# rileyhales/river-route

Hardware: AMD Instinct MI355X
Metric: reach-steps/sec (higher is better)
Workload: dtype f64

## Files before the change

### river_route_amd/csrc/rr_kernels_rec.hpp

```cpp
#pragma once

namespace {

constexpr int kRecCols = 32, kRecBatch = 8, kRecThreads = 256;
constexpr int kRecInThreads = kRecThreads, kRecOutThreads = kRecThreads;
constexpr int kRecInCols = kRecCols, kRecOutCols = kRecCols;
constexpr int kRecRows = 16 * kRecBatch;
constexpr int kRecLaunchBatches = 4, kRecMaxLaunchBatches = 8;

struct RecPermArgs {
    double *rec;
    Div32 rec_chunks;
    int64_t n, np, T, total, batch;
    Div32 nsub;
    const int2 *colmeta;
    const double *scale;
    RowView rows;
    const float *rows_in32;
    float *rows32;
    Div32 factor;
    const int32_t *cols;
    int32_t swizzle;
    int32_t clamp;
    uint32_t in32_sel, out32_sel;
// ... 23 lines not shown

constexpr int kRecTileRows = 16 * kRecBatch + 15;
constexpr int kRecTileLd = kRecCols + 1;

__device__ __forceinline__ uint32_t ring_chunk(const Div32 &chunks, uint32_t first, uint32_t ahead)
{
    const uint32_t c = first + ahead;
    return c >= chunks.d ? c - chunks.d : c;
}

template <bool SUB, int THREADS = kRecThreads, int BATCH = kRecBatch, bool LDSMETA = false, int COLS = kRecCols>
__device__ __forceinline__ void write_records(const RecPermArgs &a, const double *tile, int64_t col0, int64_t batch, int64_t tick_first, int64_t row_first,
                                              const int2 *smeta = nullptr, const double *sscale = nullptr)
{
    constexpr int R = 16 * BATCH + 15;
    const int tid = threadIdx.x;
    static_assert(COLS * BATCH * 8 % THREADS == 0, "records of a tile must divide among the threads");
    constexpr int IT = COLS * BATCH * 8 / THREADS;
    int2 meta[LDSMETA ? 1 : IT];
    double f[LDSMETA ? 1 : IT];
    if constexpr (!LDSMETA) {
#pragma unroll
        for (int it = 0; it < IT; ++it) {
            const int64_t i = col0 + (it * THREADS + tid) / (8 * BATCH);
            meta[it] = i < a.n ? a.colmeta[i] : make_int2(-1, 0);
        }
#pragma unroll
        for (int it = 0; it < IT; ++it) {
            const int64_t i = col0 + (it * THREADS + tid) / (8 * BATCH);
            f[it] = (a.scale && i < a.n) ? a.scale[i] : 1.0;
        }
    }
    const uint32_t chunk_first = a.rec_chunks.mod((uint32_t)kRecBatch * (uint32_t)batch);
#pragma unroll(LDSMETA ? (SUB ? 2 : 4) : IT)
    for (int it = 0; it < IT; ++it) {
        const int piece = it * THREADS + tid;
        const int c = piece / (8 * BATCH), k = (piece >> 3) % BATCH, part = piece & 7;
        const int2 m = LDSMETA ? smeta[c] : meta[LDSMETA ? 0 : it];
        const double scale = LDSMETA ? sscale[c] : f[LDSMETA ? 0 : it];
        const int32_t p = m.x;
        if (p < 0) continue;
        const int32_t lag = m.y & kLagMask;
        const int o = lag & 15;
        const uint32_t chunk = ring_chunk(a.rec_chunks, chunk_first, (uint32_t)(lag >> 4) + k);
        const int r = 15 - o + 16 * k + 2 * part;
        double v0, v1;
        if (SUB) {
            const int64_t t0 = tick_first + r, t1 = t0 + 1;
            uint32_t s;
            const int r0 = t0 < 0 ? 0 : (int)((int64_t)a.nsub.div((uint32_t)t0, s) - row_first);
            const int r1 = t1 < 0 ? 0 : (int)((int64_t)a.nsub.div((uint32_t)t1, s) - row_first);
            v0 = tile[min(r0, R - 1) * (COLS + 1) + c] * scale; v1 = tile[min(r1, R - 1) * (COLS + 1) + c] * scale;
        } else {
            v0 = tile[r * (COLS + 1) + c] * scale; v1 = tile[(r + 1) * (COLS + 1) + c] * scale;
        }
        double2 *dst = reinterpret_cast<double2 *>(a.rec + rec_elem(chunk, a.np, p)) + part;
        typedef double d2 __attribute__((ext_vector_type(2)));
        *reinterpret_cast<d2 *>(dst) = d2{v0, v1};
    }
}

template <bool SUB, bool IN32 = false, bool ENS = false, bool HW = false>
__global__ __launch_bounds__(kRecInThreads, 4) void k_rec_in(const RecArgsOf<ENS> args)
{
    static_assert(!HW || (!SUB && !ENS), "headwaters are routed by the in-pass only with one sub-step per row, single member");
    const RecPermArgs &a = member_args(args);
    constexpr int R = kRecTileRows, G = kRecInThreads / kRecInCols;
    __shared__ double tile[R * (kRecInCols + 1)];
    __shared__ int2 smeta[kRecInCols];
    __shared__ double sscale[kRecInCols];
    __shared__ double shw[5][HW ? kRecInCols : 1];
    const int tid = threadIdx.x;
    auto first_row = [&](int64_t tick_first) -> int64_t {
        uint32_t sub_unused;
        return SUB ? (int64_t)a.nsub.div((uint32_t)(tick_first < 0 ? 0 : tick_first), sub_unused) : tick_first;
    };
    int64_t tick_first = kRecRows * a.batch - 15;
    int64_t row_first = first_row(tick_first);
    constexpr int RPT = (R + G - 1) / G;
    const int c = tid % kRecInCols, r0 = tid / kRecInCols;
    const int need = SUB ? (int)((uint32_t)(R - 1) / a.nsub.d) + 2 : R;
    const uint32_t n_tiles = (uint32_t)((a.n + kRecInCols - 1) / kRecInCols);
    if (blockIdx.x >= n_tiles) return;
    const int64_t col0 = (int64_t)(a.swizzle ? xcd_swizzle(blockIdx.x, n_tiles) : blockIdx.x) * kRecInCols;
    const int64_t i = min(col0 + c, a.n - 1);
    const bool live = col0 + c < a.n;
    auto load = [&](int64_t t) -> double {
        const int64_t off = a.rows.offset(t < 0 ? 0 : (t >= a.T ? a.T - 1 : t)) + i;
        return IN32 ? (double)f32_from_file(a.rows_in32[off], a.in32_sel) : a.rows.base[off];
    };
    {
        double v[RPT];
        int2 cm = make_int2(-1, 0);
        double cs = 1.0;
        double hc1 = 0.0, hc2 = 0.0, hc3 = 0.0, hq = 0.0;
        if (tid < kRecInCols) {
            cm = live ? a.colmeta[i] : make_int2(-1, 0);
            cs = a.scale ? a.scale[i] : 1.0;
            if constexpr (HW) {
                hc1 = a.hw_coef[3 * i]; hc2 = a.hw_coef[3 * i + 1]; hc3 = a.hw_coef[3 * i + 2];
                hq = a.hw_carry[i];
            }
        }
#pragma unroll
        for (int q = 0; q < RPT; ++q) v[q] = load(row_first + min(r0 + q * G, need - 1));
#pragma unroll
        for (int q = 0; q < RPT; ++q) {
            const int r = r0 + q * G;
            const int64_t row = row_first + r;
            if (r < R) tile[r * (kRecInCols + 1) + c] = (row >= 0 && row < a.T && live) ? v[q] : 0.0;
        }
        if (tid < kRecInCols) {
            smeta[c] = cm; sscale[c] = cs;
            if constexpr (HW) { shw[0][c] = hc1; shw[1][c] = hc2; shw[2][c] = hc3; shw[3][c] = hq; shw[4][c] = (cm.y & kColInpass) ? 1.0 : cs; }
        }
    }
    __syncthreads();
    auto route_headwaters = [&](int64_t first) {
        if (tid >= kRecInCols) return;
        const int2 m = smeta[tid];
        if (m.x < 0 || !(m.y & kColInpass)) return;
        const double c1 = shw[0][tid], c2 = shw[1][tid], c3 = shw[2][tid], sc = sscale[tid];
        double q = shw[3][tid];
        const int r_first = 15 - (m.y & 15);
        double *col = tile + r_first * (kRecInCols + 1) + tid;
        const int64_t t_first = first + r_first;
        constexpr int kBlk = 8;
#pragma unroll 1
        for (int b = 0; b < kRecRows; b += kBlk) {
            double x[kBlk];
#pragma unroll
            for (int k = 0; k < kBlk; ++k) x[k] = col[(b + k) * (kRecInCols + 1)] * sc;
            const int64_t t0 = t_first + b;
            if (t0 >= 0 && t0 + kBlk <= a.T) {
#pragma unroll
                for (int k = 0; k < kBlk; ++k) { q = __builtin_fma(c1, 0.0, __builtin_fma(c2, 0.0, __builtin_fma(c3, q, x[k]))); x[k] = q; }
            } else {
#pragma unroll
                for (int k = 0; k < kBlk; ++k) {
                    const bool in = t0 + k >= 0 && t0 + k < a.T;
                    const double qn = __builtin_fma(c1, 0.0, __builtin_fma(c2, 0.0, __builtin_fma(c3, q, x[k])));
                    q = in ? qn : q; x[k] = in ? qn : x[k];
                }
            }
#pragma unroll
            for (int k = 0; k < kBlk; ++k) col[(b + k) * (kRecInCols + 1)] = x[k];
        }
        shw[3][tid] = q;
    };
    const double *wscale = HW ? shw[4] : sscale;
    if constexpr (HW) { route_headwaters(tick_first); __syncthreads(); }
    const int nb = a.batches > 1 ? a.batches : 1;
    for (int b = 1; b < nb; ++b) {
        constexpr int NPT = kRecRows / G, KPT = 3;
        const int64_t tick_next = tick_first + kRecRows, row_next = first_row(tick_next);
        const int shift = (int)(row_next - row_first), keep = max(need - shift, 0);
        double v[NPT], kv[KPT];
#pragma unroll
        for (int q = 0; q < NPT; ++q) {
            const int r = keep + r0 + q * G;
            if (r < need) v[q] = load(row_next + r);
        }
        write_records<SUB, kRecInThreads, kRecBatch, true, kRecInCols>(a, tile, col0, a.batch + b - 1, tick_first, row_first, smeta, wscale);
#pragma unroll
        for (int q = 0; q < KPT; ++q) {
            const int r = r0 + q * G;
            if (r < keep) kv[q] = tile[(shift + r) * (kRecInCols + 1) + c];
        }
        __syncthreads();
#pragma unroll
        for (int q = 0; q < KPT; ++q) {
            const int r = r0 + q * G;
            if (r < keep) tile[r * (kRecInCols + 1) + c] = kv[q];
        }
#pragma unroll
        for (int q = 0; q < NPT; ++q) {
            const int r = keep + r0 + q * G;
            const int64_t row = row_next + r;
            if (r < need) tile[r * (kRecInCols + 1) + c] = (row >= 0 && row < a.T && live) ? v[q] : 0.0;
        }
        __syncthreads();
        tick_first = tick_next; row_first = row_next;
        if constexpr (HW) { route_headwaters(tick_first); __syncthreads(); }
    }
    if constexpr (HW) {
        if (tid < kRecInCols && live && (smeta[tid].y & kColInpass)) a.hw_carry[i] = shw[3][tid];
    }
    write_records<SUB, kRecInThreads, kRecBatch, true, kRecInCols>(a, tile, col0, a.batch + nb - 1, tick_first, row_first, smeta, wscale);
}

struct UhArgs {
    const double *kernel, *state;
    int32_t n_ks;
};
constexpr int kUhCols = 16, kUhTileLd = kUhCols + 1;
constexpr int kUhMaxBatches = 2;
constexpr int uh_threads(int batches) { return 32 * kRecBatch * batches; }
constexpr int uh_tile_rows(int batches) { return 16 * kRecBatch * batches + 15; }
constexpr int uh_groups(int batches) { return uh_threads(batches) / kUhCols; }
constexpr int uh_rows_per_thread(int batches) { return (uh_tile_rows(batches) + uh_groups(batches) - 1) / uh_groups(batches); }
constexpr int uh_win_rows(int batches) { return uh_groups(batches) * uh_rows_per_thread(batches); }
constexpr size_t rec_in_uh_lds_bytes(int nk, int batches) { return (size_t)((uh_win_rows(batches) + nk - 1) + nk) * kUhTileLd * sizeof(double); }

template <bool SUB, int NK, int BATCHES, bool IN32 = false>
__global__ __launch_bounds__(uh_threads(BATCHES)) void k_rec_in_uh(const RecPermArgs a, const UhArgs u)
{
    constexpr int R = uh_tile_rows(BATCHES), G = uh_groups(BATCHES), RP = uh_rows_per_thread(BATCHES);
    constexpr int ROWS = uh_win_rows(BATCHES) + NK - 1, DATA = R + NK - 1;
    extern __shared__ __attribute__((aligned(16))) double uh_lds[];
    double *dt = uh_lds;
    double *tp = uh_lds + ROWS * kUhTileLd;
    const int tid = threadIdx.x, c = tid % kUhCols, g = tid / kUhCols;
    const int64_t col0 = (int64_t)(a.swizzle ? xcd_swizzle(blockIdx.x, gridDim.x) : blockIdx.x) * kUhCols;
    const int64_t tick_first = kRecRows * a.batch - 15;
    uint32_t sub_unused;
    const int64_t row_first = SUB ? (int64_t)a.nsub.div((uint32_t)(tick_first < 0 ? 0 : tick_first), sub_unused) : tick_first;
    const int need = SUB ? (int)((uint32_t)(R - 1) / a.nsub.d) + 2 : R;
    const int64_t i = min(col0 + c, a.n - 1);
    const bool live = col0 + c < a.n;
    const int32_t tb = (int32_t)row_first - (NK - 1) + g;
    {
// ... 206 lines not shown
```

### river_route_amd/csrc/rr_engine.hip

```cpp
#include "rr_common.hpp"
#include "rr_kernels_tick.hpp"
#include "rr_kernels_tile.hpp"
#include "rr_kernels_uh.hpp"
#include "rr_kernels_rec.hpp"
#include "rr_kernels_runoff.hpp"
#include "rr_kernels_direct.hpp"
#include "rr_kernels_metrics.hpp"
#include "rr_kernels_overlap.hpp"
#include "rr_kernels_adjoint.hpp"
#include "rr_kernels_adjoint_unit.hpp"
#include "rr_exec.hpp"


extern "C" {

int rr_version(void) { return RR_VERSION_NUM; }

const char *rr_last_error(void) { return g_err.c_str(); }

int rr_device_count(void)
{
    int c = 0;
    if (hipGetDeviceCount(&c) != hipSuccess) return 0;
    return c;
// ... 144 lines not shown
    info[0] = P->h.n; info[1] = P->h.n_edges; info[2] = P->h.depth; info[3] = P->h.widest_level;
    info[4] = P->h.n_headwaters; info[5] = P->h.n_outlets; info[6] = P->h.identity ? 1 : 0; info[7] = P->device;
    return RR_OK;
}

int rr_plan_layout(const rr_plan *P, int32_t *perm, int32_t *lag, int32_t *child_ptr)
{
    if (!P) return fail(RR_E_INVALID, "rr_plan_layout: null plan");
    const size_t n = (size_t)P->h.n;
    if (perm && n) std::memcpy(perm, P->h.perm.data(), n * sizeof(int32_t));
    if (lag && n) std::memcpy(lag, P->h.lag.data(), n * sizeof(int32_t));
    if (child_ptr) std::memcpy(child_ptr, P->h.child_ptr.data(), (n + 1) * sizeof(int32_t));
    return RR_OK;
}

int rr_plan_tile_info(const rr_plan *P, int64_t info[8])
{
    if (!P || !info) return fail(RR_E_INVALID, "rr_plan_tile_info: null argument");
    const rr::TilePlan &T = P->tp;
    info[0] = T.ok ? 1 : 0; info[1] = T.block; info[2] = T.np; info[3] = T.n_ghost; info[4] = T.n_tiles; info[5] = T.n_levels;
    info[6] = P->wave_threads; info[7] = kRecRows;
    return RR_OK;
}

int rr_plan_inpass_info(const rr_plan *P, int64_t info[5])
{
    if (!P || !info) return fail(RR_E_INVALID, "rr_plan_inpass_info: null argument");
    for (int k = 0; k < 5; ++k) info[k] = 0;
    info[0] = P->hw_inpass ? 1 : 0;
    if (!P->tp.ok) return RR_OK;
    std::vector<int32_t> lag(P->tp.lag);
    for (int32_t i : P->ghost_reach) lag[P->tp.inv[i]] |= kGhostBit;
    std::vector<uint8_t> elig;
    rr::mark_inpass_headwaters(P->tp, lag, kGhostBit, elig, info + 1);
    return RR_OK;
}

int rr_plan_tile_layout(const rr_plan *P, int32_t *tile_ptr, int32_t *tile_level, int32_t *perm, int32_t *lag, int32_t *cfirst,
                        uint32_t *ccnt, int32_t *xpos)
{
    if (!P) return fail(RR_E_INVALID, "rr_plan_tile_layout: null plan");
    const rr::TilePlan &T = P->tp;
    if (!T.ok) return fail(RR_E_UNSUPPORTED, "rr_plan_tile_layout: this network does not tile (a reach has more upstream reaches than a tile holds)");
    auto copy = [](auto *dst, const auto &src) { if (dst && !src.empty()) std::memcpy(dst, src.data(), src.size() * sizeof(src[0])); };
    copy(tile_ptr, T.tile_ptr); copy(tile_level, T.tile_level); copy(perm, T.perm); copy(lag, T.lag); copy(cfirst, T.cfirst);
    copy(ccnt, T.ccnt); copy(xpos, T.xpos);
    return RR_OK;
}

int rr_plan_direct_info(const rr_plan *P, int64_t info[8], char *why, int64_t why_cap)
{
    if (!P || !info) return fail(RR_E_INVALID, "rr_plan_direct_info: null argument");
    const rr::DirectPlan &D = P->dp;
    info[0] = D.ok ? 1 : 0; info[1] = D.n_tiles; info[2] = D.n_holes; info[3] = D.n_exports; info[4] = D.skel.np; info[5] = D.skel.n_tiles;
    info[6] = D.skel.n_levels; info[7] = P->direct_window;
    if (why && why_cap > 0) { std::strncpy(why, D.why.c_str(), (size_t)why_cap - 1); why[why_cap - 1] = 0; }
    return RR_OK;
}

int rr_plan_direct_layout(const rr_plan *P, int32_t *tile_c0, int32_t *tile_nc, int32_t *tile_lag_lo, int32_t *tile_span, int32_t *delay, int32_t *up3, int32_t *xinfo)
{
    if (!P) return fail(RR_E_INVALID, "rr_plan_direct_layout: null plan");
    const rr::DirectPlan &D = P->dp;
    if (!D.ok) return fail(RR_E_UNSUPPORTED, "rr_plan_direct_layout: the direct row path does not apply to this plan: " + D.why);
    auto copy = [](auto *dst, const auto &src) { if (dst && !src.empty()) std::memcpy(dst, src.data(), src.size() * sizeof(src[0])); };
    copy(tile_c0, D.tile_c0); copy(tile_nc, D.tile_nc); copy(tile_lag_lo, D.tile_lag_lo); copy(tile_span, D.tile_span);
    copy(delay, D.delay); copy(up3, D.up3); copy(xinfo, D.xinfo);
// ... 27 lines not shown
    int rc = need_device(P);
    if (rc) return rc;
    const rr::HostPlan &H = P->h;
    const int64_t n = H.n;
    if (n > 0 && (!c2 || !c3 || (H.n_edges > 0 && !lhs_off_data)))
        return fail(RR_E_INVALID, "rr_plan_set_coeffs: null coefficient array");
    std::vector<double> w(n), a2(n), a3(n), a4(n, 0.0);
    for (int64_t p = 0; p < n; ++p) {
        const int32_t i = H.perm[p];
        const int32_t e = H.edge_of[i];
        w[p] = e >= 0 ? -lhs_off_data[e] : 0.0;
        a2[p] = c2[i];
        a3[p] = c3[i];
        if (c4_dt) a4[p] = c4_dt[i];
    }
    std::vector<double> c1row(n, 0.0);
    bool uniform = true;
    for (int64_t p = 0; p < n; ++p) {
        const int32_t u0 = H.child_ptr[p], u1 = H.child_ptr[p + 1];
        if (u1 > u0) c1row[p] = w[u0];
        for (int32_t u = u0 + 1; u < u1; ++u) if (w[u] != w[u0]) uniform = false;
    }
    P->weights_uniform = uniform;
    rc = dev_upload(P->d_w, w);
    if (!rc) rc = dev_upload(P->d_c1row_h, c1row);
    if (!rc && P->tp.ok) {
        const rr::TilePlan &TP = P->tp;
        P->h_coef.assign(3 * TP.np, 0.0);
        for (int64_t p = 0; p < TP.np; ++p) {
            if (TP.lag[p] & kTileGhostBit) continue;
            const int32_t i = TP.perm[p];
            P->h_coef[3 * p] = c1row[H.inv[i]]; P->h_coef[3 * p + 1] = c2[i]; P->h_coef[3 * p + 2] = c3[i];
        }
        rc = upload_tile_coef(P);
    }
    {
        P->h_dcoef.assign(4 * (size_t)n, 0.0);
        for (int64_t i = 0; i < n; ++i) { P->h_dcoef[4 * i] = c1row[H.inv[i]]; P->h_dcoef[4 * i + 1] = c2[i]; P->h_dcoef[4 * i + 2] = c3[i]; P->h_dcoef[4 * i + 3] = c4_dt ? c4_dt[i] : 0.0; }
        if (!rc) rc = upload_direct_coef(P);
    }
    if (!rc) rc = dev_upload(P->d_c2, a2);
    if (!rc) rc = dev_upload(P->d_c3, a3);
    if (!rc) rc = dev_upload(P->d_c4, a4);
    if (!rc && c4_dt && n > 0) {
        hipError_t e = hipMemcpy(P->d_c4_params, c4_dt, (size_t)n * sizeof(double), hipMemcpyHostToDevice);
        if (e != hipSuccess) rc = fail(RR_E_HIP, hipGetErrorString(e));
    }
    if (rc) return rc;
    P->coeffs_set = true;
    P->has_c4 = c4_dt != nullptr;
    return RR_OK;
}

int rr_plan_set_unit_weights(rr_plan *P, const double *c1, const double *a_data)
{
    int rc = need_device(P);
    if (rc) return rc;
    if (P->ses.open) return fail(RR_E_STATE, "rr_plan_set_unit_weights: a routing call is open");
    if (!c1 && !a_data) { P->unit_general = false; return RR_OK; }
    const rr::HostPlan &H = P->h;
    const int64_t n = H.n;
    if (!c1 || (H.n_edges > 0 && !a_data)) return fail(RR_E_INVALID, "rr_plan_set_unit_weights: give both arrays, or neither to go back to unit weights");
    if (P->n_ghost > 0 || P->n_export > 0) return fail(RR_E_UNSUPPORTED, "rr_plan_set_unit_weights: general edge data on a partitioned network is not supported");
    std::vector<double> a2(n, 0.0), own(n, 0.0);
    for (int64_t p = 0; p < n; ++p) {
        const int32_t i = H.perm[p], e = H.edge_of[i];
        a2[p] = e >= 0 ? a_data[e] : 0.0;
// ... 1236 lines not shown
```

### river_route_amd/csrc/rr_exec.hpp

```cpp
#pragma once


enum class Mode { Rapid, Muskingum, Unit };

struct Rows {
    const double *dev_in = nullptr;
    const float *dev_in32 = nullptr;
    const double *host_in = nullptr;
    int64_t rows_in = 0;
    double *dev_out = nullptr;
    double *host_out = nullptr;
    int64_t rows_out = 0;
    float *dev_out32 = nullptr;
    int64_t out_factor = 1;
    const double *uh_kernel = nullptr, *uh_state = nullptr;
    int64_t uh_nks = 0;
    const RunoffArgs *runoff = nullptr;
    int64_t members = 0, in_pitch = 0, out_pitch = 0;
};

struct CallShape {
    Mode mode = Mode::Rapid;
    int64_t T = 0, nsub = 1;
    bool host = false;
// ... 88 lines not shown
    int32_t *d_bidx = nullptr;
    uint16_t *d_hwc = nullptr;
    double *d_w = nullptr, *d_c1row_h = nullptr, *d_c2 = nullptr, *d_c3 = nullptr, *d_c4 = nullptr;
    double *d_x = nullptr, *d_isum = nullptr, *d_qch = nullptr;
    double *d_a2 = nullptr, *d_c1own = nullptr, *d_z = nullptr;
    bool unit_general = false;
    double *d_ring = nullptr;
    int64_t ring_cap = 0;
    double *d_stage = nullptr;
    int64_t stage_cap = 0;
    double *d_mrows = nullptr;
    int64_t mrows_cap = 0;
    uint16_t *d_slot_a[2] = {nullptr, nullptr}, *d_slot_b[2] = {nullptr, nullptr};
    int32_t *d_m_index[2] = {nullptr, nullptr};
    int64_t perm_rows_per_block = 2;

    rr::TilePlan tp;
    bool wave_enabled = true, wave_forced = false, weights_uniform = false;
    bool ens_enabled = true;
    int wave_threads = 512;
    int64_t wave_K = 0;
    Schedule sch;
    int64_t kc_cap = int64_t{1} << 20;
    TileMeta *d_tmeta = nullptr;
    int4 *d_pmeta = nullptr;
    int32_t *d_tperm = nullptr, *d_tinv = nullptr;
    int32_t *d_inner_idx = nullptr;
    bool export_inside = false;
    double *d_coef = nullptr;
    double *d_coef_unit = nullptr;
    bool hw_inpass = true;
    std::vector<uint8_t> hw_elig;
    int64_t hw_counts[4] = {0, 0, 0, 0};
    int4 *d_pmeta_hw = nullptr;
    double *d_coef_hw = nullptr;
    double *d_hwcoef = nullptr;
    double *d_hwq = nullptr;
    std::vector<double> h_coef;
    int32_t n_wide_tiles = 0;
    double *d_sq = nullptr, *d_ss = nullptr, *d_si = nullptr, *d_sqch = nullptr;
    double *d_esq = nullptr, *d_ess = nullptr, *d_esi = nullptr;
    int64_t ens_cap = 0;
    double *d_full = nullptr, *d_chan = nullptr;
    int2 *d_colmeta = nullptr;
    int2 *d_ghostmeta = nullptr;
    double *d_c4_params = nullptr;
    size_t dev_total_bytes = 0;
    int cu_count = 256;

    int64_t n_ghost = 0, n_export = 0;
    int64_t ghost_min_lag = 0, export_max_lag = 0;
    std::vector<int32_t> ghost_reach, export_reach;

    Session ses;
    HostPipe pipe;
    rr::DirectPlan dp;
    bool direct_enabled = true;
    bool uh_rows_ok = true;
    int direct_window = 1;
    DirectTile *d_dtiles = nullptr;
    int4 *d_dlane = nullptr;
    int32_t *d_dsend_ptr = nullptr, *d_dsend_lane = nullptr;
    double *d_dcoef = nullptr, *d_dq = nullptr;
    TileMeta *d_ktmeta = nullptr;
    int4 *d_kpmeta = nullptr;
    int32_t *d_kperm = nullptr, *d_kholecol = nullptr;
// ... 48 lines not shown
int need_device(const rr_plan *plan)
{
    if (!plan) return fail(RR_E_INVALID, "null plan");
    if (plan->device < 0)
        return fail(RR_E_NO_DEVICE, "this plan is host-only (RR_DEVICE_NONE): the HIP engine has no CPU fallback");
    HIPCHK(hipSetDevice(plan->device));
    return RR_OK;
}

template <typename T>
int ensure_cap(T **buf, int64_t *cap, int64_t count)
{
    if (*cap >= count) return RR_OK;
    if (*buf) { (void)hipFree(*buf); *buf = nullptr; *cap = 0; }
    int rc = dev_alloc(buf, count);
    if (rc) return rc;
    *cap = count;
    return RR_OK;
}

int upload_tile_meta(rr_plan *P, const std::vector<int32_t> &lag, const std::vector<int32_t> &xpos, const std::vector<int32_t> &flags)
{
    const rr::TilePlan &TP = P->tp;
    std::vector<TileMeta> tm((size_t)TP.n_tiles);
    for (int32_t t = 0; t < TP.n_tiles; ++t)
        tm[t] = TileMeta{TP.tile_ptr[t], TP.tile_ptr[t + 1], TP.tile_level[t], TP.tile_lag_lo[t], TP.tile_lag_hi[t], flags[t], 0, 0};
    std::vector<int4> pm((size_t)TP.np);
    for (int64_t p = 0; p < TP.np; ++p) pm[p] = make_int4(lag[p], TP.cfirst[p], xpos[p], (int32_t)TP.ccnt[p]);
    int rc = RR_OK;
    if (!P->d_tmeta) rc = dev_alloc(&P->d_tmeta, TP.n_tiles);
    if (!rc && !P->d_pmeta) rc = dev_alloc(&P->d_pmeta, TP.np);
    if (!rc) rc = dev_upload(P->d_tmeta, tm);
    if (!rc) rc = dev_upload(P->d_pmeta, pm);
    rr::mark_inpass_headwaters(TP, lag, kGhostBit, P->hw_elig, P->hw_counts);
    if (!P->hw_inpass) { P->hw_elig.assign((size_t)TP.np, 0); P->hw_counts[0] = 0; }
    for (int64_t p = 0; p < TP.np; ++p) if (P->hw_elig[p]) pm[p].x |= kTileGhostBit;
    const rr::HostPlan &H = P->h;
    std::vector<int2> cm((size_t)H.n);
    for (int64_t i = 0; i < H.n; ++i)
        cm[i] = make_int2(TP.inv[i], (TP.lag[TP.inv[i]] & kLagMask) | (H.child_ptr[H.inv[i] + 1] == H.child_ptr[H.inv[i]] ? kColHeadwater : 0) |
                                         (P->hw_elig[TP.inv[i]] ? kColInpass : 0));
    if (!rc && !P->d_pmeta_hw) rc = dev_alloc(&P->d_pmeta_hw, TP.np);
    if (!rc) rc = dev_upload(P->d_pmeta_hw, pm);
    if (!rc && !P->d_colmeta) rc = dev_alloc(&P->d_colmeta, H.n);
    if (!rc) rc = dev_upload(P->d_colmeta, cm);
    return rc;
}

int upload_tile_coef(rr_plan *P)
{
    if (P->h_coef.empty()) return RR_OK;
    std::vector<double> coef(P->h_coef);
    for (int32_t i : P->ghost_reach) { const int64_t p = P->tp.inv[i]; coef[3 * p] = coef[3 * p + 1] = coef[3 * p + 2] = 0.0; }
    int rc = dev_upload(P->d_coef, coef);
    if (rc) return rc;
    {
        std::vector<double> hw(coef);
        for (int64_t p = 0; p < P->tp.np; ++p)
            if (P->hw_elig[p]) hw[3 * p] = hw[3 * p + 1] = hw[3 * p + 2] = 0.0;
        rc = dev_upload(P->d_coef_hw, hw);
        if (rc) return rc;
        std::vector<double> col(3 * (size_t)P->h.n);
        for (int64_t i = 0; i < P->h.n; ++i) for (int k = 0; k < 3; ++k) col[3 * i + k] = coef[3 * (int64_t)P->tp.inv[i] + k];
        rc = dev_upload(P->d_hwcoef, col);
        if (rc) return rc;
    }
    for (int64_t p = 0; p < P->tp.np; ++p)
// ... 1364 lines not shown
```

### river_route_amd/csrc/rr_plan.cpp

```cpp
#include "rr_plan.hpp"

#include <algorithm>
#include <cstdlib>
#include <limits>
#include <utility>
#include <vector>

#include "../../include/rr_hip.h"

namespace rr {

void build_tiled_permutation(const int32_t *pi, int64_t n, int32_t tile, TiledPermutation &T)
{
    T = TiledPermutation();
    T.n = n;
    T.tile = tile;
    if (n == 0) return;
    const int64_t nt = (n + tile - 1) / tile;
    std::vector<int32_t> q_of(n);
    for (int64_t q = 0; q < n; ++q) q_of[pi[q]] = (int32_t)q;
    std::vector<int64_t> run(nt * nt + 1, 0);
    for (int64_t i = 0; i < n; ++i) ++run[(int64_t)(q_of[i] / tile) * nt + i / tile + 1];
    for (size_t k = 1; k < run.size(); ++k) run[k] += run[k - 1];
    std::vector<int32_t> g_of(n);
    for (int64_t i = 0; i < n; ++i) g_of[i] = (int32_t)run[(int64_t)(q_of[i] / tile) * nt + i / tile]++;
    T.slot_a.resize(n); T.m_index.resize(n); T.slot_b.resize(n);
    std::vector<std::pair<int32_t, int32_t>> tmp;
    for (int64_t a = 0; a < nt; ++a) {
        const int64_t i0 = a * tile, i1 = std::min<int64_t>(n, i0 + tile);
        tmp.clear();
        for (int64_t i = i0; i < i1; ++i) tmp.emplace_back(g_of[i], (int32_t)i);
        std::sort(tmp.begin(), tmp.end());
        for (size_t m = 0; m < tmp.size(); ++m) {
            T.slot_a[tmp[m].second] = (uint16_t)m;
            T.m_index[i0 + (int64_t)m] = tmp[m].first;
        }
// ... 290 lines not shown
                    if (is_hw(c) != (pass == 0)) continue;
                    const bool ghost = tile_of_reach[c] != t;
                    T.perm.push_back(c);
                    T.lag.push_back(lag_of[c] | (ghost ? kTileGhost : 0));
                    if (ghost) ghost_positions.push_back((int32_t)T.perm.size() - 1);
                    ++cnt; if (pass == 0) ++hw;
                }
            T.ccnt.push_back(cnt | (hw << 16));
        }
        int32_t lo = std::numeric_limits<int32_t>::max(), hi = 0;
        for (int64_t p = base; p < (int64_t)T.perm.size(); ++p) { const int32_t l = T.lag[p] & (kTileExport - 1); lo = std::min(lo, l); hi = std::max(hi, l); }
        T.tile_lag_lo[t] = lo; T.tile_lag_hi[t] = hi;
        if ((int64_t)T.perm.size() - base > block) return;
    }
    T.np = (int64_t)T.perm.size();
    T.tile_ptr[n_tiles] = (int32_t)T.np;
    T.tile_flags.assign(n_tiles, 0);
    for (int32_t t = 0; t < n_tiles; ++t)
        for (int32_t p = T.tile_ptr[t]; p < T.tile_ptr[t + 1]; ++p)
            if ((T.ccnt[p] & 0xFFFFu) > 3) { T.tile_flags[t] = 1; break; }
    T.n_ghost = (int64_t)ghost_positions.size();
    T.xpos.assign(T.np, -1);
    T.tile_of.assign(T.np, 0);
    for (int32_t t = 0; t < n_tiles; ++t) for (int32_t p = T.tile_ptr[t]; p < T.tile_ptr[t + 1]; ++p) T.tile_of[p] = t;
    if (skeleton_only) T.ext_ghost.assign(n, -1);
    for (int32_t g : ghost_positions) {
        const int32_t src = T.inv[T.perm[g]];
        if (src < 0) { T.ext_ghost[T.perm[g]] = g; continue; }
        T.xpos[g] = src; T.xpos[src] = g; T.lag[src] |= kTileExport;
    }
    T.ok = true;
}

int64_t mark_inpass_headwaters(const TilePlan &T, const std::vector<int32_t> &lag, int32_t boundary_ghost, std::vector<uint8_t> &eligible, int64_t counts[4])
{
    eligible.assign((size_t)T.np, 0);
    int64_t c[4] = {0, 0, 0, 0};
    for (int64_t p = 0; p < T.np; ++p) {
        if ((lag[p] & kTileGhost) || (T.ccnt[p] & 0xFFFFu) != 0) continue;
        ++c[1];
        if (lag[p] & (kTileExport | boundary_ghost)) { ++c[2]; continue; }
        if (T.tile_flags[T.tile_of[p]] & 1) { ++c[3]; continue; }
        eligible[p] = 1;
        ++c[0];
    }
    if (counts) for (int k = 0; k < 4; ++k) counts[k] = c[k];
    return c[0];
}

void build_direct_plan(const std::vector<int32_t> &down, const std::vector<int32_t> &lag_of, int32_t lanes, int32_t wmax, int32_t skel_block,
                       DirectPlan &D, const std::vector<uint8_t> *ghost, const std::vector<int32_t> *export_slot)
{
    D = DirectPlan();
    D.lanes = lanes; D.wmax = wmax;
    const int64_t n = (int64_t)down.size();
    if (n == 0) { D.why = "empty network"; return; }
    if (lanes > 1023) { D.why = "more lanes than a lane number holds"; return; }
    std::vector<int32_t> sub(n, 1), height(n, 1), first(n), indeg(n, 0);
    for (int64_t v = 0; v < n; ++v) first[v] = (int32_t)v;
    for (int64_t c = 0; c < n; ++c)
        if (down[c] >= 0) {
            const int32_t d = down[c];
            sub[d] += sub[c]; height[d] = std::max(height[d], height[c] + 1); first[d] = std::min(first[d], first[c]); ++indeg[d];
        }
    D.big.assign(n, 0);
    for (int64_t v = 0; v < n; ++v) D.big[v] = (sub[v] > lanes || height[v] > wmax) ? 1 : 0;
    auto small_root = [&](int64_t v) { return !D.big[v] && (down[v] < 0 || D.big[down[v]]); };
    auto is_ghost = [&](int64_t v) { return ghost && (*ghost)[v] != 0; };
    if (ghost)
        for (int64_t v = 0; v < n; ++v)
            if (is_ghost(v)) for (int64_t w = down[v]; w >= 0 && !D.big[w]; w = down[w]) D.big[w] = 1;
    for (int64_t v = 0; v < n; ++v) {
        if (is_ghost(v) && (indeg[v] != 0 || down[v] < 0)) { D.why = "a boundary ghost is not a headwater with a downstream reach"; return; }
        if (export_slot && (*export_slot)[v] >= 0 && down[v] >= 0) { D.why = "a boundary export has a downstream reach in this plan"; return; }
        if (D.big[v]) continue;
// ... 234 lines not shown
```

### river_route_amd/csrc/rr_plan.hpp

```cpp
#pragma once
#include <cstdint>
#include <string>
#include <vector>

namespace rr {

struct HostPlan {
    int64_t n = 0;
    int64_t n_edges = 0;
    int32_t depth = 0;
    int64_t widest_level = 0;
    int64_t n_headwaters = 0;
    int64_t n_outlets = 0;
    bool identity = false;

    std::vector<int32_t> perm;
    std::vector<int32_t> inv;
    std::vector<int32_t> lag;
    std::vector<int32_t> child_ptr;
    std::vector<uint16_t> hw_children;
    std::vector<int64_t> lag_start;
    std::vector<int32_t> edge_of;
    std::vector<int32_t> inner_pos;
    std::vector<int32_t> down;
// ... 7 lines not shown
    std::vector<uint16_t> slot_b;
};
void build_tiled_permutation(const int32_t *pi, int64_t n, int32_t tile, TiledPermutation &out);

void partition_forest(const std::vector<int32_t> &down, int32_t n_parts, int32_t *part_of, std::vector<int64_t> &sizes);


constexpr int32_t kTileGhost = 1 << 28;
constexpr int32_t kTileExport = 1 << 27;
struct TilePlan {
    bool ok = false;
    int32_t block = 0;
    int64_t np = 0;
    int64_t n_ghost = 0;
    int32_t n_tiles = 0, n_levels = 0;
    std::vector<int32_t> tile_ptr;
    std::vector<int32_t> tile_level;
    std::vector<int32_t> tile_lag_lo, tile_lag_hi;
    std::vector<int32_t> tile_flags;
    std::vector<int32_t> level_start;
    std::vector<int32_t> perm;
    std::vector<int32_t> inv;
    std::vector<int32_t> lag;
    std::vector<int32_t> cfirst;
    std::vector<uint32_t> ccnt;
    std::vector<int32_t> xpos;
    std::vector<int32_t> tile_of;
    std::vector<int32_t> ext_ghost;
};
void build_tile_plan(const std::vector<int32_t> &down, const std::vector<int32_t> &lag_of, int32_t block, TilePlan &out,
                     const std::vector<uint8_t> *big = nullptr, bool skeleton_only = false);

int64_t mark_inpass_headwaters(const TilePlan &tp, const std::vector<int32_t> &lag, int32_t boundary_ghost, std::vector<uint8_t> &eligible,
                               int64_t counts[4] = nullptr);

constexpr int32_t kDirectHole = 1 << 30;
constexpr int32_t kDirectSenderShift = 8, kDirectDelayMask = 0xFF;
constexpr int32_t kDirectExport = 1 << 15;
struct DirectPlan {
    bool ok = false;
    std::string why;
    int32_t lanes = 0, wmax = 0;
    int32_t n_tiles = 0;
    int64_t n_holes = 0, n_exports = 0;
    std::vector<int32_t> tile_c0, tile_nc, tile_lag_lo, tile_span;
    std::vector<int32_t> delay;
    std::vector<int32_t> up3;
    std::vector<int32_t> xinfo;
    std::vector<uint8_t> big;
    std::vector<int32_t> send_ptr;
    std::vector<int32_t> send_lane;
    TilePlan skel;
};
constexpr int32_t kDirectSenders = 64;
void build_direct_plan(const std::vector<int32_t> &down, const std::vector<int32_t> &lag_of, int32_t lanes, int32_t wmax, int32_t skel_block,
                       DirectPlan &out, const std::vector<uint8_t> *ghost = nullptr, const std::vector<int32_t> *export_slot = nullptr);

bool postorder(const int64_t *down, int64_t n, int64_t *order);

int build_host_plan(int64_t n, const int32_t *indptr, const int32_t *indices, HostPlan &plan, std::string &err);

}
```

Before: 129.2 billion.

## Overlap headwater routing with plain-column record writes via wave specialization

In the headwater in-pass kernel, the first wave now routes the headwater columns while the remaining three waves write records for the non-routed columns at the same time. A compacted per-tile list of routed and plain columns is built with ballots, so the record writes skip dead columns. Routed columns are written by all threads after a barrier. This removes the serialized route-then-sync-then-write step, at the cost of extra LDS lists, more barriers and a specialized write path that assumes no sub-stepping.

```diff
diff --git a/river_route_amd/csrc/rr_kernels_rec.hpp b/river_route_amd/csrc/rr_kernels_rec.hpp
--- a/river_route_amd/csrc/rr_kernels_rec.hpp
+++ b/river_route_amd/csrc/rr_kernels_rec.hpp
@@ -107,6 +107,28 @@
     }
 }
 
+template <int THREADS>
+__device__ __forceinline__ void write_records_list(const RecPermArgs &a, const double *tile, uint32_t chunk_first, const unsigned char *list, int count, int t,
+                                                   const int2 *smeta, const double *sscale)
+{
+    static_assert(THREADS % 8 == 0, "a record is written by 8 consecutive lanes");
+    const int pieces = count * 8 * kRecBatch;
+#pragma unroll 2
+    for (int piece = t; piece < pieces; piece += THREADS) {
+        const int c = list[piece / (8 * kRecBatch)], k = (piece >> 3) % kRecBatch, part = piece & 7;
+        const int2 m = smeta[c];
+        const double scale = sscale[c];
+        const int32_t lag = m.y & kLagMask;
+        const int o = lag & 15;
+        const uint32_t chunk = ring_chunk(a.rec_chunks, chunk_first, (uint32_t)(lag >> 4) + k);
+        const int r = 15 - o + 16 * k + 2 * part;
+        const double v0 = tile[r * kRecTileLd + c] * scale, v1 = tile[(r + 1) * kRecTileLd + c] * scale;
+        double2 *dst = reinterpret_cast<double2 *>(a.rec + rec_elem(chunk, a.np, m.x)) + part;
+        typedef double d2 __attribute__((ext_vector_type(2)));
+        *reinterpret_cast<d2 *>(dst) = d2{v0, v1};
+    }
+}
+
 template <bool SUB, bool IN32 = false, bool ENS = false, bool HW = false>
 __global__ __launch_bounds__(kRecInThreads, 4) void k_rec_in(const RecArgsOf<ENS> args)
 {
@@ -117,6 +139,8 @@
     __shared__ int2 smeta[kRecInCols];
     __shared__ double sscale[kRecInCols];
     __shared__ double shw[5][HW ? kRecInCols : 1];
+    __shared__ unsigned char slist[2][HW ? kRecInCols : 1];
+    __shared__ int scount[2];
     const int tid = threadIdx.x;
     auto first_row = [&](int64_t tick_first) -> int64_t {
         uint32_t sub_unused;
@@ -159,7 +183,14 @@
         }
         if (tid < kRecInCols) {
             smeta[c] = cm; sscale[c] = cs;
-            if constexpr (HW) { shw[0][c] = hc1; shw[1][c] = hc2; shw[2][c] = hc3; shw[3][c] = hq; shw[4][c] = (cm.y & kColInpass) ? 1.0 : cs; }
+            if constexpr (HW) {
+                shw[0][c] = hc1; shw[1][c] = hc2; shw[2][c] = hc3; shw[3][c] = hq; shw[4][c] = (cm.y & kColInpass) ? 1.0 : cs;
+                const bool alive = cm.x >= 0, routed = alive && (cm.y & kColInpass);
+                const unsigned long long mr = __ballot(routed), mp = __ballot(alive && !routed), below = (1ull << c) - 1;
+                if (routed) slist[0][__popcll(mr & below)] = (unsigned char)c;
+                else if (alive) slist[1][__popcll(mp & below)] = (unsigned char)c;
+                if (c == 0) { scount[0] = __popcll(mr); scount[1] = __popcll(mp); }
+            }
         }
     }
     __syncthreads();
@@ -196,19 +227,33 @@
         shw[3][tid] = q;
     };
     const double *wscale = HW ? shw[4] : sscale;
-    if constexpr (HW) { route_headwaters(tick_first); __syncthreads(); }
+    constexpr int kWave = 64, kPlainThreads = kRecInThreads - kWave;
+    auto write_plain = [&](int64_t batch) {
+        if (tid >= kWave)
+            write_records_list<kPlainThreads>(a, tile, a.rec_chunks.mod((uint32_t)kRecBatch * (uint32_t)batch), slist[1], scount[1], tid - kWave, smeta, wscale);
+    };
+    auto write_routed = [&](int64_t batch) {
+        write_records_list<kRecInThreads>(a, tile, a.rec_chunks.mod((uint32_t)kRecBatch * (uint32_t)batch), slist[0], scount[0], tid, smeta, wscale);
+    };
     const int nb = a.batches > 1 ? a.batches : 1;
     for (int b = 1; b < nb; ++b) {
         constexpr int NPT = kRecRows / G, KPT = 3;
         const int64_t tick_next = tick_first + kRecRows, row_next = first_row(tick_next);
         const int shift = (int)(row_next - row_first), keep = max(need - shift, 0);
         double v[NPT], kv[KPT];
+        if constexpr (HW) { if (tid < kWave) route_headwaters(tick_first); }
 #pragma unroll
         for (int q = 0; q < NPT; ++q) {
             const int r = keep + r0 + q * G;
             if (r < need) v[q] = load(row_next + r);
         }
-        write_records<SUB, kRecInThreads, kRecBatch, true, kRecInCols>(a, tile, col0, a.batch + b - 1, tick_first, row_first, smeta, wscale);
+        if constexpr (HW) {
+            write_plain(a.batch + b - 1);
+            __syncthreads();
+            write_routed(a.batch + b - 1);
+        } else {
+            write_records<SUB, kRecInThreads, kRecBatch, true, kRecInCols>(a, tile, col0, a.batch + b - 1, tick_first, row_first, smeta, wscale);
+        }
 #pragma unroll
         for (int q = 0; q < KPT; ++q) {
             const int r = r0 + q * G;
@@ -228,12 +273,16 @@
         }
         __syncthreads();
         tick_first = tick_next; row_first = row_next;
-        if constexpr (HW) { route_headwaters(tick_first); __syncthreads(); }
     }
     if constexpr (HW) {
-        if (tid < kRecInCols && live && (smeta[tid].y & kColInpass)) a.hw_carry[i] = shw[3][tid];
-    }
-    write_records<SUB, kRecInThreads, kRecBatch, true, kRecInCols>(a, tile, col0, a.batch + nb - 1, tick_first, row_first, smeta, wscale);
+        if (tid < kWave) route_headwaters(tick_first);
+        write_plain(a.batch + nb - 1);
+        if (tid < kRecInCols && smeta[tid].x >= 0 && (smeta[tid].y & kColInpass)) a.hw_carry[col0 + tid] = shw[3][tid];
+        __syncthreads();
+        write_routed(a.batch + nb - 1);
+    } else {
+        write_records<SUB, kRecInThreads, kRecBatch, true, kRecInCols>(a, tile, col0, a.batch + nb - 1, tick_first, row_first, smeta, wscale);
+    }
 }
 
 struct UhArgs {
```

New measurement: 131.4 billion, median of 6. 1.7% higher.

## Simplify in-pass headwater routing to the c3 recurrence and restrict eligibility

Applied to the files above, without the earlier changes.

The in-pass headwater recurrence drops the c1/c2 terms, which were multiplied by zero inflow, and keeps only the c3 term, so a headwater needs fewer coefficient loads and less shared memory. Eligibility now also requires c1 to be exactly zero and c2 to be finite, and tile metadata is re-uploaded once coefficients are set so the eligibility uses real coefficients. The input tile loader now derives column and row group from thread bits, has every thread load its own metadata, and drops the live and row-bound guards in favour of a padded tile. The record writer fully unrolls in the LDS-metadata path and skips the negative-column check there. The trade-off is some headwaters falling back to the regular path, plus the cost of keeping metadata copies for re-upload.

```diff
diff --git a/river_route_amd/csrc/rr_engine.hip b/river_route_amd/csrc/rr_engine.hip
--- a/river_route_amd/csrc/rr_engine.hip
+++ b/river_route_amd/csrc/rr_engine.hip
@@ -200,7 +200,7 @@
     std::vector<int32_t> lag(P->tp.lag);
     for (int32_t i : P->ghost_reach) lag[P->tp.inv[i]] |= kGhostBit;
     std::vector<uint8_t> elig;
-    rr::mark_inpass_headwaters(P->tp, lag, kGhostBit, elig, info + 1);
+    rr::mark_inpass_headwaters(P->tp, lag, kGhostBit, elig, info + 1, P->h_coef.empty() ? nullptr : P->h_coef.data());
     return RR_OK;
 }
 
@@ -294,7 +294,8 @@
             const int32_t i = TP.perm[p];
             P->h_coef[3 * p] = c1row[H.inv[i]]; P->h_coef[3 * p + 1] = c2[i]; P->h_coef[3 * p + 2] = c3[i];
         }
-        rc = upload_tile_coef(P);
+        if (!P->meta_lag.empty()) rc = upload_tile_meta(P, P->meta_lag, P->meta_xpos, P->meta_flags);
+        if (!rc) rc = upload_tile_coef(P);
     }
     {
         P->h_dcoef.assign(4 * (size_t)n, 0.0);
diff --git a/river_route_amd/csrc/rr_exec.hpp b/river_route_amd/csrc/rr_exec.hpp
--- a/river_route_amd/csrc/rr_exec.hpp
+++ b/river_route_amd/csrc/rr_exec.hpp
@@ -144,6 +144,7 @@
     bool hw_inpass = true;
     std::vector<uint8_t> hw_elig;
     int64_t hw_counts[4] = {0, 0, 0, 0};
+    std::vector<int32_t> meta_lag, meta_xpos, meta_flags;
     int4 *d_pmeta_hw = nullptr;
     double *d_coef_hw = nullptr;
     double *d_hwcoef = nullptr;
@@ -258,7 +259,8 @@
     if (!rc && !P->d_pmeta) rc = dev_alloc(&P->d_pmeta, TP.np);
     if (!rc) rc = dev_upload(P->d_tmeta, tm);
     if (!rc) rc = dev_upload(P->d_pmeta, pm);
-    rr::mark_inpass_headwaters(TP, lag, kGhostBit, P->hw_elig, P->hw_counts);
+    rr::mark_inpass_headwaters(TP, lag, kGhostBit, P->hw_elig, P->hw_counts, P->h_coef.empty() ? nullptr : P->h_coef.data());
+    if (&lag != &P->meta_lag) { P->meta_lag = lag; P->meta_xpos = xpos; P->meta_flags = flags; }
     if (!P->hw_inpass) { P->hw_elig.assign((size_t)TP.np, 0); P->hw_counts[0] = 0; }
     for (int64_t p = 0; p < TP.np; ++p) if (P->hw_elig[p]) pm[p].x |= kTileGhostBit;
     const rr::HostPlan &H = P->h;
diff --git a/river_route_amd/csrc/rr_kernels_rec.hpp b/river_route_amd/csrc/rr_kernels_rec.hpp
--- a/river_route_amd/csrc/rr_kernels_rec.hpp
+++ b/river_route_amd/csrc/rr_kernels_rec.hpp
@@ -79,14 +79,14 @@
         }
     }
     const uint32_t chunk_first = a.rec_chunks.mod((uint32_t)kRecBatch * (uint32_t)batch);
-#pragma unroll(LDSMETA ? (SUB ? 2 : 4) : IT)
+#pragma unroll(LDSMETA ? (SUB ? 2 : IT) : IT)
     for (int it = 0; it < IT; ++it) {
         const int piece = it * THREADS + tid;
         const int c = piece / (8 * BATCH), k = (piece >> 3) % BATCH, part = piece & 7;
         const int2 m = LDSMETA ? smeta[c] : meta[LDSMETA ? 0 : it];
         const double scale = LDSMETA ? sscale[c] : f[LDSMETA ? 0 : it];
         const int32_t p = m.x;
-        if (p < 0) continue;
+        if (!LDSMETA && p < 0) continue;
         const int32_t lag = m.y & kLagMask;
         const int o = lag & 15;
         const uint32_t chunk = ring_chunk(a.rec_chunks, chunk_first, (uint32_t)(lag >> 4) + k);
@@ -107,16 +107,20 @@
     }
 }
 
+__device__ __forceinline__ int32_t fresh_tid(int32_t v) { asm volatile("" : "+v"(v)); return v; }
+
 template <bool SUB, bool IN32 = false, bool ENS = false, bool HW = false>
 __global__ __launch_bounds__(kRecInThreads, 4) void k_rec_in(const RecArgsOf<ENS> args)
 {
     static_assert(!HW || (!SUB && !ENS), "headwaters are routed by the in-pass only with one sub-step per row, single member");
     const RecPermArgs &a = member_args(args);
     constexpr int R = kRecTileRows, G = kRecInThreads / kRecInCols;
-    __shared__ double tile[R * (kRecInCols + 1)];
+    constexpr int RPT = (R + G - 1) / G;
+    static_assert((kRecInCols & (kRecInCols - 1)) == 0 && (G & (G - 1)) == 0, "column and row group of a thread are bit fields of its number");
+    __shared__ double tile[RPT * G * (kRecInCols + 1)];
     __shared__ int2 smeta[kRecInCols];
     __shared__ double sscale[kRecInCols];
-    __shared__ double shw[5][HW ? kRecInCols : 1];
+    __shared__ double shw[3][HW ? kRecInCols : 1];
     const int tid = threadIdx.x;
     auto first_row = [&](int64_t tick_first) -> int64_t {
         uint32_t sub_unused;
@@ -124,53 +128,47 @@
     };
     int64_t tick_first = kRecRows * a.batch - 15;
     int64_t row_first = first_row(tick_first);
-    constexpr int RPT = (R + G - 1) / G;
-    const int c = tid % kRecInCols, r0 = tid / kRecInCols;
     const int need = SUB ? (int)((uint32_t)(R - 1) / a.nsub.d) + 2 : R;
     const uint32_t n_tiles = (uint32_t)((a.n + kRecInCols - 1) / kRecInCols);
     if (blockIdx.x >= n_tiles) return;
     const int64_t col0 = (int64_t)(a.swizzle ? xcd_swizzle(blockIdx.x, n_tiles) : blockIdx.x) * kRecInCols;
-    const int64_t i = min(col0 + c, a.n - 1);
-    const bool live = col0 + c < a.n;
-    auto load = [&](int64_t t) -> double {
+    auto col_of = [&](int t) -> int64_t { return min(col0 + (t & (kRecInCols - 1)), a.n - 1); };
+    auto group_of = [](int t) -> int { return (t / kRecInCols) & (G - 1); };
+    auto load = [&](int64_t t, int64_t i) -> double {
         const int64_t off = a.rows.offset(t < 0 ? 0 : (t >= a.T ? a.T - 1 : t)) + i;
         return IN32 ? (double)f32_from_file(a.rows_in32[off], a.in32_sel) : a.rows.base[off];
     };
     {
+        const int c = tid & (kRecInCols - 1), r0 = group_of(tid);
+        const int64_t i = col_of(tid);
         double v[RPT];
-        int2 cm = make_int2(-1, 0);
-        double cs = 1.0;
-        double hc1 = 0.0, hc2 = 0.0, hc3 = 0.0, hq = 0.0;
-        if (tid < kRecInCols) {
-            cm = live ? a.colmeta[i] : make_int2(-1, 0);
-            cs = a.scale ? a.scale[i] : 1.0;
-            if constexpr (HW) {
-                hc1 = a.hw_coef[3 * i]; hc2 = a.hw_coef[3 * i + 1]; hc3 = a.hw_coef[3 * i + 2];
-                hq = a.hw_carry[i];
-            }
-        }
-#pragma unroll
-        for (int q = 0; q < RPT; ++q) v[q] = load(row_first + min(r0 + q * G, need - 1));
+        const int2 cm = a.colmeta[i];
+        const double cs = a.scale ? a.scale[i] : 1.0;
+        double hc3 = 0.0, hq = 0.0;
+        if constexpr (HW) { hc3 = a.hw_coef[3 * i + 2]; hq = a.hw_carry[i]; }
+#pragma unroll
+        for (int q = 0; q < RPT; ++q) v[q] = load(row_first + min(r0 + q * G, need - 1), i);
 #pragma unroll
         for (int q = 0; q < RPT; ++q) {
             const int r = r0 + q * G;
             const int64_t row = row_first + r;
-            if (r < R) tile[r * (kRecInCols + 1) + c] = (row >= 0 && row < a.T && live) ? v[q] : 0.0;
+            tile[r * (kRecInCols + 1) + c] = (row >= 0 && row < a.T) ? v[q] : 0.0;
         }
         if (tid < kRecInCols) {
             smeta[c] = cm; sscale[c] = cs;
-            if constexpr (HW) { shw[0][c] = hc1; shw[1][c] = hc2; shw[2][c] = hc3; shw[3][c] = hq; shw[4][c] = (cm.y & kColInpass) ? 1.0 : cs; }
+            if constexpr (HW) { shw[0][c] = hc3; shw[1][c] = hq; shw[2][c] = (cm.y & kColInpass) ? 1.0 : cs; }
         }
     }
     __syncthreads();
     auto route_headwaters = [&](int64_t first) {
-        if (tid >= kRecInCols) return;
-        const int2 m = smeta[tid];
-        if (m.x < 0 || !(m.y & kColInpass)) return;
-        const double c1 = shw[0][tid], c2 = shw[1][tid], c3 = shw[2][tid], sc = sscale[tid];
-        double q = shw[3][tid];
+        const int t = fresh_tid(tid);
+        if (t >= kRecInCols) return;
+        const int2 m = smeta[t];
+        if (!(m.y & kColInpass)) return;
+        const double c3 = shw[0][t], sc = sscale[t];
+        double q = shw[1][t];
         const int r_first = 15 - (m.y & 15);
-        double *col = tile + r_first * (kRecInCols + 1) + tid;
+        double *col = tile + r_first * (kRecInCols + 1) + t;
         const int64_t t_first = first + r_first;
         constexpr int kBlk = 8;
 #pragma unroll 1
@@ -181,32 +179,36 @@
             const int64_t t0 = t_first + b;
             if (t0 >= 0 && t0 + kBlk <= a.T) {
 #pragma unroll
-                for (int k = 0; k < kBlk; ++k) { q = __builtin_fma(c1, 0.0, __builtin_fma(c2, 0.0, __builtin_fma(c3, q, x[k]))); x[k] = q; }
+                for (int k = 0; k < kBlk; ++k) { q = __builtin_fma(c3, q, x[k]) + 0.0; x[k] = q; }
             } else {
 #pragma unroll
                 for (int k = 0; k < kBlk; ++k) {
                     const bool in = t0 + k >= 0 && t0 + k < a.T;
-                    const double qn = __builtin_fma(c1, 0.0, __builtin_fma(c2, 0.0, __builtin_fma(c3, q, x[k])));
+                    const double qn = __builtin_fma(c3, q, x[k]) + 0.0;
                     q = in ? qn : q; x[k] = in ? qn : x[k];
                 }
             }
 #pragma unroll
             for (int k = 0; k < kBlk; ++k) col[(b + k) * (kRecInCols + 1)] = x[k];
         }
-        shw[3][tid] = q;
+        shw[1][t] = q;
     };
-    const double *wscale = HW ? shw[4] : sscale;
+    const double *wscale = HW ? shw[2] : sscale;
     if constexpr (HW) { route_headwaters(tick_first); __syncthreads(); }
     const int nb = a.batches > 1 ? a.batches : 1;
     for (int b = 1; b < nb; ++b) {
         constexpr int NPT = kRecRows / G, KPT = 3;
         const int64_t tick_next = tick_first + kRecRows, row_next = first_row(tick_next);
         const int shift = (int)(row_next - row_first), keep = max(need - shift, 0);
+        const int t = fresh_tid(tid), c = t & (kRecInCols - 1), r0 = group_of(t);
         double v[NPT], kv[KPT];
-#pragma unroll
-        for (int q = 0; q < NPT; ++q) {
-            const int r = keep + r0 + q * G;
-            if (r < need) v[q] = load(row_next + r);
+        {
+            const int64_t i = col_of(t);
+#pragma unroll
+            for (int q = 0; q < NPT; ++q) {
+                const int r = keep + r0 + q * G;
+                if (!SUB || r < need) v[q] = load(row_next + r, i);
+            }
         }
         write_records<SUB, kRecInThreads, kRecBatch, true, kRecInCols>(a, tile, col0, a.batch + b - 1, tick_first, row_first, smeta, wscale);
 #pragma unroll
@@ -224,14 +226,15 @@
         for (int q = 0; q < NPT; ++q) {
             const int r = keep + r0 + q * G;
             const int64_t row = row_next + r;
-            if (r < need) tile[r * (kRecInCols + 1) + c] = (row >= 0 && row < a.T && live) ? v[q] : 0.0;
+            if (!SUB || r < need) tile[r * (kRecInCols + 1) + c] = (row >= 0 && row < a.T) ? v[q] : 0.0;
         }
         __syncthreads();
         tick_first = tick_next; row_first = row_next;
         if constexpr (HW) { route_headwaters(tick_first); __syncthreads(); }
     }
     if constexpr (HW) {
-        if (tid < kRecInCols && live && (smeta[tid].y & kColInpass)) a.hw_carry[i] = shw[3][tid];
+        const int t = fresh_tid(tid);
+        if (t < kRecInCols && col0 + t < a.n && (smeta[t].y & kColInpass)) a.hw_carry[col0 + t] = shw[1][t];
     }
     write_records<SUB, kRecInThreads, kRecBatch, true, kRecInCols>(a, tile, col0, a.batch + nb - 1, tick_first, row_first, smeta, wscale);
 }
diff --git a/river_route_amd/csrc/rr_plan.cpp b/river_route_amd/csrc/rr_plan.cpp
--- a/river_route_amd/csrc/rr_plan.cpp
+++ b/river_route_amd/csrc/rr_plan.cpp
@@ -1,7 +1,9 @@
 #include "rr_plan.hpp"
 
 #include <algorithm>
+#include <cstdint>
 #include <cstdlib>
+#include <cstring>
 #include <limits>
 #include <utility>
 #include <vector>
@@ -358,15 +360,21 @@
     T.ok = true;
 }
 
-int64_t mark_inpass_headwaters(const TilePlan &T, const std::vector<int32_t> &lag, int32_t boundary_ghost, std::vector<uint8_t> &eligible, int64_t counts[4])
+int64_t mark_inpass_headwaters(const TilePlan &T, const std::vector<int32_t> &lag, int32_t boundary_ghost, std::vector<uint8_t> &eligible, int64_t counts[4],
+                               const double *coef)
 {
     eligible.assign((size_t)T.np, 0);
     int64_t c[4] = {0, 0, 0, 0};
+    auto bits = [](double x) { uint64_t u; std::memcpy(&u, &x, sizeof u); return u; };
+    auto plain_coef = [&](int64_t p) {
+        return bits(coef[3 * p]) == 0 && (bits(coef[3 * p + 1]) & 0x7FF0000000000000ull) != 0x7FF0000000000000ull;
+    };
     for (int64_t p = 0; p < T.np; ++p) {
         if ((lag[p] & kTileGhost) || (T.ccnt[p] & 0xFFFFu) != 0) continue;
         ++c[1];
         if (lag[p] & (kTileExport | boundary_ghost)) { ++c[2]; continue; }
         if (T.tile_flags[T.tile_of[p]] & 1) { ++c[3]; continue; }
+        if (coef && !plain_coef(p)) continue;
         eligible[p] = 1;
         ++c[0];
     }
diff --git a/river_route_amd/csrc/rr_plan.hpp b/river_route_amd/csrc/rr_plan.hpp
--- a/river_route_amd/csrc/rr_plan.hpp
+++ b/river_route_amd/csrc/rr_plan.hpp
@@ -63,7 +63,7 @@
                      const std::vector<uint8_t> *big = nullptr, bool skeleton_only = false);
 
 int64_t mark_inpass_headwaters(const TilePlan &tp, const std::vector<int32_t> &lag, int32_t boundary_ghost, std::vector<uint8_t> &eligible,
-                               int64_t counts[4] = nullptr);
+                               int64_t counts[4] = nullptr, const double *coef = nullptr);
 
 constexpr int32_t kDirectHole = 1 << 30;
 constexpr int32_t kDirectSenderShift = 8, kDirectDelayMask = 0xFF;
```

New measurement: 129.8 billion before, 132.9 billion after (median of 6 runs). 2.4% higher.
